# shangzhouye/stereo-visual-slam

Hardware: AMD Instinct MI355X
Metric: stereo keyframes/sec (ORB+match+tri+local-BA), KITTI-00 1241x376 (higher is better)
Workload: dtype u8+f64

## Files before the change

### stereo-visual-slam_amd/csrc/match_kernels.hip

```cpp
#include "vslam_internal.h"

namespace vslam {

typedef int v4i __attribute__((ext_vector_type(4)));
typedef int v16i __attribute__((ext_vector_type(16)));

__device__ inline uint32_t expand_nibble(uint32_t nib) {
    const uint32_t s = __umul24(nib & 0xFu, 0x204081u) & 0x01010101u;
    return ((s << 8) - (s << 1)) | 0x01010101u;
}
__device__ inline int4 expand_half(uint32_t bits16) {
    return make_int4((int)expand_nibble(bits16), (int)expand_nibble(bits16 >> 4), (int)expand_nibble(bits16 >> 8), (int)expand_nibble(bits16 >> 12));
}

constexpr int kMatchBlock = 256;
constexpr int kColTiles = 4;
constexpr int kColsPerWave = 32 * kColTiles;
constexpr int kColsPerBlock = (kMatchBlock / 64) * kColsPerWave;
constexpr int kQRows = 32;
constexpr int kQStride = 272;

__device__ inline void fold_tile(const v16i (&acc)[kColTiles], int ib, int nq, bool full, int (&m)[kColTiles]) {
    const int inv = 0xFFFF - ib;
    if (full) {
#pragma unroll
        for (int v = 0; v < 16; ++v) {
            const int iv = inv - (8 * (v / 4) + (v % 4));
#pragma unroll
            for (int t = 0; t < kColTiles; ++t) m[t] = max(m[t], (acc[t][v] << 16) + iv);
        }
    } else {
#pragma unroll
        for (int v = 0; v < 16; ++v) {
            const int off = 8 * (v / 4) + (v % 4);
            if (ib + off < nq) {
#pragma unroll
                for (int t = 0; t < kColTiles; ++t) m[t] = max(m[t], (acc[t][v] << 16) + inv - off);
            }
        }
    }
}

template <bool kSel>
__global__ __launch_bounds__(kMatchBlock) void match_train_nearest_kernel(
    const uint8_t* __restrict__ d_q, size_t q_stride, const int32_t* __restrict__ d_nq, const uint8_t* __restrict__ d_t, size_t t_stride,
    const int32_t* __restrict__ d_nt, int max_rows, int qsplit, int B, uint32_t* __restrict__ d_train_best, const int32_t* __restrict__ d_qsel,
    int sel_cap, const int32_t* __restrict__ d_nqsel) {
    const int w = blockIdx.x;
    const int b = w % B, split = (w / B) % qsplit, cb = w / (B * qsplit);
    const int nrows = min(d_nq[b], max_rows), nt = min(d_nt[b], max_rows);
    const int nq = kSel ? min(max(d_nqsel[b], 0), min(sel_cap, nrows)) : nrows;
    const int32_t* sel = kSel ? d_qsel + (size_t)b * sel_cap : nullptr;
    const int c0 = cb * kColsPerBlock;
    if (c0 >= nt || nq <= 0) return;
    const int ntiles = (nq + kQRows - 1) / kQRows, per = (ntiles + qsplit - 1) / qsplit;
    const int tile0 = split * per, tile1 = min(ntiles, tile0 + per);
    if (tile0 >= tile1) return;
    const int lane = threadIdx.x & 63, wave = threadIdx.x >> 6, r = lane & 31, h = lane >> 5;
    __shared__ alignas(16) int8_t sq[2][kQRows * kQStride];
    __shared__ uint2 lut[256];
    {
        const uint32_t v = threadIdx.x;
        lut[v] = make_uint2(expand_nibble(v), expand_nibble(v >> 4));
    }
    const uint8_t* Q = d_q + (size_t)b * q_stride;
    const uint8_t* T = d_t + (size_t)b * t_stride;
    v4i breg[kColTiles][8];
#pragma unroll
    for (int t = 0; t < kColTiles; ++t) {
        const int j = min(c0 + wave * kColsPerWave + 32 * t + r, nt - 1);
        const uint4 lo = *reinterpret_cast<const uint4*>(T + (size_t)j * 32), hi = *reinterpret_cast<const uint4*>(T + (size_t)j * 32 + 16);
        const uint32_t wd[8] = {lo.x, lo.y, lo.z, lo.w, hi.x, hi.y, hi.z, hi.w};
#pragma unroll
        for (int s = 0; s < 8; ++s) {
            const int4 e = expand_half((wd[s] >> (16 * h)) & 0xFFFFu);
            breg[t][s] = v4i{e.x, e.y, e.z, e.w};
        }
    }
    const int srow = threadIdx.x >> 3, sword = threadIdx.x & 7;
    auto gload = [&](int tile, uint32_t& x) {
        int r0 = min(tile * kQRows + srow, nq - 1);
        if (kSel) r0 = min(max(sel[r0], 0), nrows - 1);
        x = reinterpret_cast<const uint32_t*>(Q + (size_t)r0 * 32)[sword];
    };
    auto sstore = [&](int buf, uint32_t x) {
        const uint2 b0 = lut[x & 0xFFu], b1 = lut[(x >> 8) & 0xFFu], b2 = lut[(x >> 16) & 0xFFu], b3 = lut[x >> 24];
        int4* dst = reinterpret_cast<int4*>(&sq[buf][srow * kQStride + sword * 32]);
        dst[0] = make_int4((int)b0.x, (int)b0.y, (int)b1.x, (int)b1.y); dst[1] = make_int4((int)b2.x, (int)b2.y, (int)b3.x, (int)b3.y);
    };
    auto mma_tile = [&](int buf, v16i (&acc)[kColTiles]) {
        v4i a[8];
#pragma unroll
        for (int s = 0; s < 8; ++s) a[s] = *reinterpret_cast<const v4i*>(&sq[buf][r * kQStride + s * 32 + h * 16]);
        const v16i zero = {0, 0, 0, 0, 0, 0, 0, 0, 0, 0, 0, 0, 0, 0, 0, 0};
#pragma unroll
        for (int t = 0; t < kColTiles; ++t) acc[t] = __builtin_amdgcn_mfma_i32_32x32x32_i8(a[0], breg[t][0], zero, 0, 0, 0);
#pragma unroll
        for (int s = 1; s < 8; ++s)
#pragma unroll
            for (int t = 0; t < kColTiles; ++t) acc[t] = __builtin_amdgcn_mfma_i32_32x32x32_i8(a[s], breg[t][s], acc[t], 0, 0, 0);
    };
    uint32_t x;
    gload(tile0, x);
    __syncthreads();
    sstore(0, x);
    if (tile0 + 1 < tile1) gload(tile0 + 1, x);
    __syncthreads();
    int m[kColTiles];
#pragma unroll
    for (int t = 0; t < kColTiles; ++t) m[t] = INT_MIN;
    v16i acc[kColTiles];
    for (int tile = tile0; tile < tile1; ++tile) {
        const int buf = (tile - tile0) & 1;
        if (tile + 1 < tile1) { sstore(buf ^ 1, x); if (tile + 2 < tile1) gload(tile + 2, x); }
        mma_tile(buf, acc);
        fold_tile(acc, tile * kQRows + 4 * h, nq, tile * kQRows + kQRows <= nq, m);
        __syncthreads();
    }
#pragma unroll
    for (int t = 0; t < kColTiles; ++t) m[t] = max(m[t], __shfl_xor(m[t], 32));
    if (h == 0) {
#pragma unroll
        for (int t = 0; t < kColTiles; ++t) {
            const int mm = m[t];
            const int j = c0 + wave * kColsPerWave + 32 * t + r;
            if (j < nt && mm != INT_MIN) {
                const uint32_t d = (uint32_t)(256 - (mm >> 16)) >> 1, i = 0xFFFFu - ((uint32_t)mm & 0xFFFFu);
                const uint32_t key = (d << 16) | i;
                if (qsplit == 1) d_train_best[(size_t)b * max_rows + j] = key;
                else atomicMin(&d_train_best[(size_t)b * max_rows + j], key);
            }
        }
    }
}

__device__ inline int block_rank(bool flag, int* s_wave_tot, int& total) {
    const int lane = threadIdx.x & 63, wave = threadIdx.x >> 6, nwaves = blockDim.x >> 6;
    const unsigned long long m = __ballot(flag);
    const int rank = __popcll(m & ((1ull << lane) - 1ull));
    __syncthreads();
    if (lane == 0) s_wave_tot[wave] = __popcll(m);
    __syncthreads();
    int base = 0, tot = 0;
    for (int w = 0; w < nwaves; ++w) {
        const int c = s_wave_tot[w];
        if (w < wave) base += c;
        tot += c;
    }
    total = tot;
    return base + rank;
}

constexpr int kFinBlock = 1024;

__global__ __launch_bounds__(kFinBlock) void match_finalize_kernel(
    const int32_t* __restrict__ d_nq, const int32_t* __restrict__ d_nt, const double* __restrict__ d_gap, int gate,
    double ratio, double gap_thr, int max_rows, const uint32_t* __restrict__ d_train_best, vslam_dmatch* __restrict__ d_out,
    int out_capacity, int32_t* __restrict__ d_nout, const int32_t* __restrict__ d_qsel, int sel_cap, const int32_t* __restrict__ d_nqsel) {
    const int b = blockIdx.x;
    const int nrows = min(d_nq[b], max_rows), nt = min(d_nt[b], max_rows);
    const int32_t* sel = d_qsel ? d_qsel + (size_t)b * sel_cap : nullptr;
    const int nq = sel ? min(max(d_nqsel[b], 0), min(sel_cap, nrows)) : nrows;
    __shared__ uint32_t qbest[kMaxRows];
    __shared__ int s_wave_tot[kFinBlock / 64];
    __shared__ uint32_t s_min[kFinBlock / 64];
    for (int i = threadIdx.x; i < kMaxRows; i += kFinBlock) qbest[i] = 0xFFFFFFFFu;
    __syncthreads();
    if (nq > 0)
        for (int j = threadIdx.x; j < nt; j += kFinBlock) {
            const uint32_t key = d_train_best[(size_t)b * max_rows + j];
            if (key != 0xFFFFFFFFu) atomicMin(&qbest[key & 0xFFFFu], (key & 0xFFFF0000u) | (uint32_t)j);
        }
    __syncthreads();
    uint32_t dmin = 0xFFFFu;
    for (int i = threadIdx.x; i < nq; i += kFinBlock) {
        const uint32_t key = qbest[i];
        if (key != 0xFFFFFFFFu) dmin = min(dmin, key >> 16);
    }
    for (int o = 32; o > 0; o >>= 1) dmin = min(dmin, (uint32_t)__shfl_xor((int)dmin, o));
    if ((threadIdx.x & 63) == 0) s_min[threadIdx.x >> 6] = dmin;
    __syncthreads();
    dmin = 0xFFFFu;
    for (int w = 0; w < kFinBlock / 64; ++w) dmin = min(dmin, s_min[w]);
    const double a = ratio * (double)(float)dmin, g = gap_thr * d_gap[b];
    const double thr = a > g ? a : g;
    vslam_dmatch* out = d_out + (size_t)b * out_capacity;
    int written = 0;
    for (int base = 0; base < nq; base += kFinBlock) {
        const int i = base + threadIdx.x;
        uint32_t key = 0xFFFFFFFFu;
        if (i < nq) key = qbest[i];
        bool keep = key != 0xFFFFFFFFu;
        const uint32_t d = key >> 16;
        if (keep && gate) keep = (double)(float)d <= thr;
        int total;
        const int r = block_rank(keep, s_wave_tot, total);
        if (keep && written + r < out_capacity) {
            vslam_dmatch m;
            m.queryIdx = sel ? sel[i] : i; m.trainIdx = (int)(key & 0xFFFFu); m.imgIdx = 0; m.distance = (float)d;
            out[written + r] = m;
        }
        written += total;
    }
    if (threadIdx.x == 0) d_nout[b] = min(written, out_capacity);
}

int launch_match(const uint8_t* d_q, size_t q_stride, const int32_t* d_nq, const uint8_t* d_t, size_t t_stride,
                 const int32_t* d_nt, const double* d_gap, int gate, double ratio, double gap_thr, int B, int max_rows,
                 uint32_t* d_train_best, vslam_dmatch* d_out, int out_capacity, int32_t* d_nout, hipStream_t stream, const int32_t* d_qsel, int sel_cap,
                 const int32_t* d_nqsel) {
    if (B <= 0) return VSLAM_OK;
    if (max_rows > kMaxRows || max_rows <= 0) { set_error("matcher: max_rows %d out of range (<= %d)", max_rows, kMaxRows); return VSLAM_ERR_ARG; }
    const int tblocks = (max_rows + kColsPerBlock - 1) / kColsPerBlock;
    int qsplit = 1;
    while (qsplit < 16 && (long)tblocks * qsplit * B < 1024 && max_rows / (qsplit * 2) >= 4 * kQRows) qsplit *= 2;
    if (qsplit > 1) VS_HIP(hipMemsetAsync(d_train_best, 0xFF, (size_t)B * max_rows * sizeof(uint32_t), stream));
    if (d_qsel) {
        ProfScope prof__(stream, "match_train_nearest_sel_kernel");
        hipLaunchKernelGGL(match_train_nearest_kernel<true>, dim3(tblocks * qsplit * B), dim3(kMatchBlock), 0, stream, d_q, q_stride, d_nq, d_t, t_stride,
                           d_nt, max_rows, qsplit, B, d_train_best, d_qsel, sel_cap, d_nqsel);
    } else {
        ProfScope prof__(stream, "match_train_nearest_kernel");
        hipLaunchKernelGGL(match_train_nearest_kernel<false>, dim3(tblocks * qsplit * B), dim3(kMatchBlock), 0, stream, d_q, q_stride, d_nq, d_t, t_stride,
                           d_nt, max_rows, qsplit, B, d_train_best, nullptr, 0, nullptr);
    }
    ProfScope prof__(stream, "match_finalize_kernel");
    hipLaunchKernelGGL(match_finalize_kernel, dim3(B), dim3(kFinBlock), 0, stream, d_nq, d_nt, d_gap, gate, ratio, gap_thr,
                       max_rows, d_train_best, d_out, out_capacity, d_nout, d_qsel, sel_cap, d_nqsel);
    VS_HIP(hipGetLastError());
    return VSLAM_OK;
}

}
```

Measured before the change: 61400.

## Compute Hamming distances with FP4 scaled MFMA and fold row index into f32 accumulator

Replaces the int8 32x32x32 MFMA Hamming-distance path with the gfx950 scaled f8f6f4 MFMA in FP4 mode, packing each descriptor bit into a ±1-like FP4 nibble. This halves the K-steps and shared-memory footprint and removes the byte LUT. The argmax row tie-break is encoded in the accumulator's fractional bits through the initial C operand, with a running offset per tile, replacing the integer shift-add fold. It also adds a launch-bounds occupancy hint. In exchange it relies on exact f32 arithmetic for the key encoding, which limits rows to 4096, and adds correctness risk in the index reconstruction.

```diff
diff --git a/stereo-visual-slam_amd/csrc/match_kernels.hip b/stereo-visual-slam_amd/csrc/match_kernels.hip
--- a/stereo-visual-slam_amd/csrc/match_kernels.hip
+++ b/stereo-visual-slam_amd/csrc/match_kernels.hip
@@ -3,14 +3,23 @@
 namespace vslam {
 
 typedef int v4i __attribute__((ext_vector_type(4)));
-typedef int v16i __attribute__((ext_vector_type(16)));
-
-__device__ inline uint32_t expand_nibble(uint32_t nib) {
-    const uint32_t s = __umul24(nib & 0xFu, 0x204081u) & 0x01010101u;
-    return ((s << 8) - (s << 1)) | 0x01010101u;
-}
-__device__ inline int4 expand_half(uint32_t bits16) {
-    return make_int4((int)expand_nibble(bits16), (int)expand_nibble(bits16 >> 4), (int)expand_nibble(bits16 >> 8), (int)expand_nibble(bits16 >> 12));
+typedef int v8i __attribute__((ext_vector_type(8)));
+typedef float v16f __attribute__((ext_vector_type(16)));
+
+__device__ inline v4i expand32(uint32_t x) {
+    return v4i{(int)(((x << 3) & 0x88888888u) | 0x22222222u), (int)(((x << 2) & 0x88888888u) | 0x22222222u),
+               (int)(((x << 1) & 0x88888888u) | 0x22222222u), (int)((x & 0x88888888u) | 0x22222222u)};
+}
+constexpr int kBlockScale = 0;
+__device__ inline v16f mma_fp4(v4i a, v4i b, v16f c) {
+    return __builtin_amdgcn_mfma_scale_f32_32x32x64_f8f6f4(v8i{a[0], a[1], a[2], a[3], 0, 0, 0, 0}, v8i{b[0], b[1], b[2], b[3], 0, 0, 0, 0}, c, 4, 4, 0,
+                                                           kBlockScale, 0, kBlockScale);
+}
+
+__device__ inline int fresh_tid() {
+    int t = threadIdx.x;
+    asm volatile("" : "+v"(t));
+    return t;
 }
 
 constexpr int kMatchBlock = 256;
@@ -18,31 +27,13 @@
 constexpr int kColsPerWave = 32 * kColTiles;
 constexpr int kColsPerBlock = (kMatchBlock / 64) * kColsPerWave;
 constexpr int kQRows = 32;
-constexpr int kQStride = 272;
-
-__device__ inline void fold_tile(const v16i (&acc)[kColTiles], int ib, int nq, bool full, int (&m)[kColTiles]) {
-    const int inv = 0xFFFF - ib;
-    if (full) {
-#pragma unroll
-        for (int v = 0; v < 16; ++v) {
-            const int iv = inv - (8 * (v / 4) + (v % 4));
-#pragma unroll
-            for (int t = 0; t < kColTiles; ++t) m[t] = max(m[t], (acc[t][v] << 16) + iv);
-        }
-    } else {
-#pragma unroll
-        for (int v = 0; v < 16; ++v) {
-            const int off = 8 * (v / 4) + (v % 4);
-            if (ib + off < nq) {
-#pragma unroll
-                for (int t = 0; t < kColTiles; ++t) m[t] = max(m[t], (acc[t][v] << 16) + inv - off);
-            }
-        }
-    }
-}
+constexpr int kQStride = 144;
+constexpr float kRowUnit = 1.f / 4096.f;
+constexpr float kNoRow = -4194304.f;
+static_assert(kMaxRows <= 4096, "the f32 key holds the row in 12 fraction bits");
 
 template <bool kSel>
-__global__ __launch_bounds__(kMatchBlock) void match_train_nearest_kernel(
+__global__ __launch_bounds__(kMatchBlock, 3) void match_train_nearest_kernel(
     const uint8_t* __restrict__ d_q, size_t q_stride, const int32_t* __restrict__ d_nq, const uint8_t* __restrict__ d_t, size_t t_stride,
     const int32_t* __restrict__ d_nt, int max_rows, int qsplit, int B, uint32_t* __restrict__ d_train_best, const int32_t* __restrict__ d_qsel,
     int sel_cap, const int32_t* __restrict__ d_nqsel) {
@@ -58,74 +49,72 @@
     if (tile0 >= tile1) return;
     const int lane = threadIdx.x & 63, wave = threadIdx.x >> 6, r = lane & 31, h = lane >> 5;
     __shared__ alignas(16) int8_t sq[2][kQRows * kQStride];
-    __shared__ uint2 lut[256];
-    {
-        const uint32_t v = threadIdx.x;
-        lut[v] = make_uint2(expand_nibble(v), expand_nibble(v >> 4));
-    }
     const uint8_t* Q = d_q + (size_t)b * q_stride;
     const uint8_t* T = d_t + (size_t)b * t_stride;
-    v4i breg[kColTiles][8];
+    v4i breg[kColTiles][4];
 #pragma unroll
     for (int t = 0; t < kColTiles; ++t) {
         const int j = min(c0 + wave * kColsPerWave + 32 * t + r, nt - 1);
-        const uint4 lo = *reinterpret_cast<const uint4*>(T + (size_t)j * 32), hi = *reinterpret_cast<const uint4*>(T + (size_t)j * 32 + 16);
-        const uint32_t wd[8] = {lo.x, lo.y, lo.z, lo.w, hi.x, hi.y, hi.z, hi.w};
-#pragma unroll
-        for (int s = 0; s < 8; ++s) {
-            const int4 e = expand_half((wd[s] >> (16 * h)) & 0xFFFFu);
-            breg[t][s] = v4i{e.x, e.y, e.z, e.w};
-        }
+        const uint4 d = *reinterpret_cast<const uint4*>(T + (size_t)j * 32 + 16 * h);
+        breg[t][0] = expand32(d.x); breg[t][1] = expand32(d.y); breg[t][2] = expand32(d.z); breg[t][3] = expand32(d.w);
     }
     const int srow = threadIdx.x >> 3, sword = threadIdx.x & 7;
     auto gload = [&](int tile, uint32_t& x) {
         int r0 = min(tile * kQRows + srow, nq - 1);
         if (kSel) r0 = min(max(sel[r0], 0), nrows - 1);
-        x = reinterpret_cast<const uint32_t*>(Q + (size_t)r0 * 32)[sword];
+        x = *reinterpret_cast<const uint32_t*>(Q + ((uint32_t)r0 * 32u + (uint32_t)sword * 4u));
     };
-    auto sstore = [&](int buf, uint32_t x) {
-        const uint2 b0 = lut[x & 0xFFu], b1 = lut[(x >> 8) & 0xFFu], b2 = lut[(x >> 16) & 0xFFu], b3 = lut[x >> 24];
-        int4* dst = reinterpret_cast<int4*>(&sq[buf][srow * kQStride + sword * 32]);
-        dst[0] = make_int4((int)b0.x, (int)b0.y, (int)b1.x, (int)b1.y); dst[1] = make_int4((int)b2.x, (int)b2.y, (int)b3.x, (int)b3.y);
-    };
-    auto mma_tile = [&](int buf, v16i (&acc)[kColTiles]) {
-        v4i a[8];
-#pragma unroll
-        for (int s = 0; s < 8; ++s) a[s] = *reinterpret_cast<const v4i*>(&sq[buf][r * kQStride + s * 32 + h * 16]);
-        const v16i zero = {0, 0, 0, 0, 0, 0, 0, 0, 0, 0, 0, 0, 0, 0, 0, 0};
-#pragma unroll
-        for (int t = 0; t < kColTiles; ++t) acc[t] = __builtin_amdgcn_mfma_i32_32x32x32_i8(a[0], breg[t][0], zero, 0, 0, 0);
-#pragma unroll
-        for (int s = 1; s < 8; ++s)
-#pragma unroll
-            for (int t = 0; t < kColTiles; ++t) acc[t] = __builtin_amdgcn_mfma_i32_32x32x32_i8(a[s], breg[t][s], acc[t], 0, 0, 0);
-    };
+    auto sstore = [&](int buf, uint32_t x) { *reinterpret_cast<v4i*>(&sq[buf][srow * kQStride + sword * 16]) = expand32(x); };
+    v16f ctie;
+#pragma unroll
+    for (int v = 0; v < 16; ++v) ctie[v] = (float)(31 - (8 * (v / 4) + (v % 4) + 4 * h)) * kRowUnit;
     uint32_t x;
     gload(tile0, x);
-    __syncthreads();
     sstore(0, x);
     if (tile0 + 1 < tile1) gload(tile0 + 1, x);
     __syncthreads();
-    int m[kColTiles];
-#pragma unroll
-    for (int t = 0; t < kColTiles; ++t) m[t] = INT_MIN;
-    v16i acc[kColTiles];
+    float m[kColTiles];
+#pragma unroll
+    for (int t = 0; t < kColTiles; ++t) m[t] = -INFINITY;
+    v16f acc[kColTiles];
     for (int tile = tile0; tile < tile1; ++tile) {
         const int buf = (tile - tile0) & 1;
         if (tile + 1 < tile1) { sstore(buf ^ 1, x); if (tile + 2 < tile1) gload(tile + 2, x); }
-        mma_tile(buf, acc);
-        fold_tile(acc, tile * kQRows + 4 * h, nq, tile * kQRows + kQRows <= nq, m);
+        if (tile * kQRows + kQRows > nq) {
+            const int row0 = tile * kQRows + 4 * ((fresh_tid() >> 5) & 1);
+#pragma unroll
+            for (int v = 0; v < 16; ++v)
+                if (row0 + 8 * (v / 4) + (v % 4) >= nq) ctie[v] = kNoRow;
+        }
+        v4i a[4];
+#pragma unroll
+        for (int s = 0; s < 4; ++s) a[s] = *reinterpret_cast<const v4i*>(&sq[buf][r * kQStride + (4 * h + s) * 16]);
+#pragma unroll
+        for (int t = 0; t < kColTiles; ++t) acc[t] = mma_fp4(a[0], breg[t][0], ctie);
+#pragma unroll
+        for (int s = 1; s < 4; ++s)
+#pragma unroll
+            for (int t = 0; t < kColTiles; ++t) acc[t] = mma_fp4(a[s], breg[t][s], acc[t]);
+#pragma unroll
+        for (int t = 0; t < kColTiles; ++t) {
+            float mm = m[t] + 32.f * kRowUnit;
+#pragma unroll
+            for (int v = 0; v < 16; v += 2) mm = __builtin_fmaxf(__builtin_fmaxf(acc[t][v], acc[t][v + 1]), mm);
+            m[t] = mm;
+        }
         __syncthreads();
     }
 #pragma unroll
-    for (int t = 0; t < kColTiles; ++t) m[t] = max(m[t], __shfl_xor(m[t], 32));
-    if (h == 0) {
+    for (int t = 0; t < kColTiles; ++t) m[t] = __builtin_fmaxf(m[t], __shfl_xor(m[t], 32));
+    const int tid = fresh_tid();
+    if ((tid & 32) == 0) {
 #pragma unroll
         for (int t = 0; t < kColTiles; ++t) {
-            const int mm = m[t];
-            const int j = c0 + wave * kColsPerWave + 32 * t + r;
-            if (j < nt && mm != INT_MIN) {
-                const uint32_t d = (uint32_t)(256 - (mm >> 16)) >> 1, i = 0xFFFFu - ((uint32_t)mm & 0xFFFFu);
+            const float mm = m[t];
+            const int j = c0 + (tid >> 6) * kColsPerWave + 32 * t + (tid & 31);
+            if (j < nt && mm >= -256.f) {
+                const float fl = __builtin_floorf(mm);
+                const uint32_t d = (uint32_t)(256 - (int)fl) >> 1, i = (uint32_t)(32 * tile1 - 1 - (int)((mm - fl) * 4096.f));
                 const uint32_t key = (d << 16) | i;
                 if (qsplit == 1) d_train_best[(size_t)b * max_rows + j] = key;
                 else atomicMin(&d_train_best[(size_t)b * max_rows + j], key);
```

Result: faster. 63430 (median of 6 runs) (+3.3%).
